# senyuanfan/inr-for-audio

Measured on AMD Instinct MI355X. Metric: coord-samples/sec trained, SIREN 5×1024 bf16 at 1/2/4/8 MI355X; recon SNR dB, higher is better.
Workload: dtype fp16

## Files before the change

include/siren_hip.h:

```cpp
#ifndef SIREN_HIP_H
#define SIREN_HIP_H

#include <stddef.h>
#include <stdint.h>

#ifdef __cplusplus
extern "C" {
#endif

#define SIREN_ABI_VERSION 12
#define SIREN_MAX_INNER 16
#define SIREN_MAX_HIDDEN 4096
#define SIREN_ROW_TILE 128
#define SIREN_TILEQ_INTS 768

enum siren_status {
  SIREN_OK = 0,
  SIREN_ERR_SHAPE = 1001,
  SIREN_ERR_NULL = 1002,
  SIREN_ERR_CONFIG = 1003
};

int siren_abi_version(void);
const char* siren_build_id(void);
int64_t siren_struct_size(int32_t which);
const char* siren_status_string(int status);

typedef struct siren_opt_state {
  double lr, best, step;
  int32_t num_bad, last_epoch;
  double min_lr, factor, threshold, eps_lr;
  int32_t patience, pad0;
  double beta1, beta2, eps;
} siren_opt_state;

typedef struct siren_guard {
  int32_t flag;
// ... 272 lines not shown
                          void* stream);
int siren_kan_regrid_refit(const double* gram, int32_t in, int32_t out, int32_t g_old, int32_t g_new,
                           const float* spline_w, const float* scaler, float* spline_w_new, int32_t* status,
                           void* stream);
int64_t siren_kan_grid_pass_rows(int32_t in);
int64_t siren_kan_grid_workspace_bytes(int64_t rows, int32_t in);
int siren_kan_grid_knots(const float* q, int32_t in, double margin, double grid_eps, float* grid_new, void* stream);
int siren_kan_grid_gram(const float* x, int64_t rows, int32_t in, const float* grid_old, const float* grid_new,
                        int32_t accumulate, double* gram, void* ws, void* stream);
int siren_kan_grid_refit(const double* gram, int32_t in, int32_t out, const float* spline_w, const float* scaler,
                         float* spline_w_new, int32_t* status, void* ws, void* stream);

enum siren_prof_kind {
  SIREN_PROF_FIRST_FWD = 0, SIREN_PROF_INNER_FWD = 1, SIREN_PROF_HEAD = 2, SIREN_PROF_BWD_DW = 3,
  SIREN_PROF_BWD_DX = 4, SIREN_PROF_BWD_DX0 = 5, SIREN_PROF_REDUCE = 6, SIREN_PROF_UPDATE = 7,
  SIREN_PROF_KAN_FWD = 8, SIREN_PROF_KAN_DW = 9, SIREN_PROF_KAN_DX = 10, SIREN_PROF_KAN_MISC = 11,
  SIREN_PROF_HEAD_FWD = 12,
  SIREN_PROF_LOSS = 13,
  SIREN_PROF_NKINDS = 14
};
enum siren_option {
  SIREN_OPT_NT_TILE = 0, SIREN_OPT_TN_TILE = 1, SIREN_OPT_NT_PIPE = 2, SIREN_OPT_TN_PIPE = 3,
  SIREN_OPT_NT_GRID = 4, SIREN_OPT_NT_DIAG = 6, SIREN_OPT_NT_QUEUE = 8, SIREN_OPT_HEAD_FUSE = 9,
  SIREN_OPT_HB_FAULT = 10, SIREN_OPT_KAN_GENERAL = 11
};
int siren_set_option(int32_t option, int32_t value);
int siren_profile_enable(int32_t max_records);
int siren_profile_reset(void);
int siren_profile_mask(uint32_t kinds);
int siren_profile_read(int32_t kind, double* total_ms, int64_t* count);

#ifdef __cplusplus
}
#endif
#endif
```

inr-for-audio_amd/_lib.py:

```python
from __future__ import annotations

import contextlib
import ctypes
import enum
import os

import torch

_HERE = os.path.dirname(os.path.abspath(__file__))
LIB_PATH = os.path.join(_HERE, "libsiren_hip.so")
ABI_VERSION = 12
MAX_INNER = 16
MAX_HIDDEN = 4096
ROW_TILE = 128
TILEQ_INTS = 768
ACT_SINE, ACT_SNAKE, ACT_TANH = 0, 1, 2
FP32_IDENTITY, FP32_SIN, FP32_TANH, FP32_SNAKE = 0, 1, 2, 3

_p = ctypes.c_void_p
_f32p = ctypes.POINTER(ctypes.c_float)
_i32 = ctypes.c_int32
_i64 = ctypes.c_int64


class SirenOptState(ctypes.Structure):
    _fields_ = [
        ("lr", ctypes.c_double), ("best", ctypes.c_double), ("step", ctypes.c_double),
        ("num_bad", _i32), ("last_epoch", _i32),
        ("min_lr", ctypes.c_double), ("factor", ctypes.c_double),
        ("threshold", ctypes.c_double), ("eps_lr", ctypes.c_double),
        ("patience", _i32), ("pad0", _i32),
        ("beta1", ctypes.c_double), ("beta2", ctypes.c_double), ("eps", ctypes.c_double),
    ]


class SirenGuard(ctypes.Structure):
    _fields_ = [("flag", _i32), ("headroom", _i32), ("clean", _i32), ("overflows", _i32),
                ("headroom0", _i32), ("stalls", _i32)]
# ... 255 lines not shown
    for k, st in enumerate(STRUCTS):
        if lib.siren_struct_size(k) != ctypes.sizeof(st):
            raise SirenError(f"{st.__name__}: ctypes size {ctypes.sizeof(st)} != C size {lib.siren_struct_size(k)}")
    return lib


def check(status: int, what: str = "siren") -> None:
    if status != 0:
        msg = load().siren_status_string(status)
        raise SirenError(f"{what} failed with status {status}: {msg.decode() if msg else '?'}")


class Opt(enum.IntEnum):
    NT_TILE = 0
    TN_TILE = 1
    NT_PIPE = 2
    TN_PIPE = 3
    NT_GRID = 4
    NT_DIAG = 6
    NT_QUEUE = 8
    HEAD_FUSE = 9
    HB_FAULT = 10
    KAN_GENERAL = 11


OPT_DEFAULTS = {Opt.NT_TILE: 0, Opt.TN_TILE: 0, Opt.NT_PIPE: -1, Opt.TN_PIPE: -1, Opt.NT_GRID: 0,
                Opt.NT_DIAG: 0, Opt.NT_QUEUE: 1, Opt.HEAD_FUSE: 1, Opt.HB_FAULT: 0, Opt.KAN_GENERAL: 0}


def _opt_shadow(lib) -> dict:
    return lib.__dict__.setdefault("_opt_shadow", dict(OPT_DEFAULTS))


def set_option(lib, opt, value: int) -> None:
    opt = Opt(opt)
    check(lib.siren_set_option(opt, value), f"siren_set_option({opt.name}, {value})")
    _opt_shadow(lib)[opt] = value


@contextlib.contextmanager
def options(lib, values: dict):
    shadow = _opt_shadow(lib)
    with contextlib.ExitStack() as undo:
        for opt, value in values.items():
            before = shadow[Opt(opt)]
            set_option(lib, opt, value)
            undo.callback(set_option, lib, opt, before)
        yield


# ... 11 lines not shown
```

inr-for-audio_amd/csrc/capi.hip:

```cpp
#include <string.h>
#include <vector>
#include "../../include/siren_hip.h"
#include "siren_kernels.h"

using namespace siren;

static_assert(sizeof(siren_opt_state) == sizeof(OptState), "opt state layout");
static_assert(sizeof(siren_guard) == sizeof(GuardState), "guard layout");
static_assert(SIREN_TILEQ_INTS == kTileqInts, "tile-queue set size");
static_assert(SIREN_MAX_INNER == siren::kMaxInner, "max hidden layers");
static_assert((int)SIREN_FP32_SNAKE == (int)siren::FP32_SNAKE && (int)SIREN_FP32_SIN == (int)siren::FP32_SIN &&
                  (int)SIREN_FP32_TANH == (int)siren::FP32_TANH, "fp32 act codes");

namespace {

inline hipStream_t S(void* s) { return (hipStream_t)s; }
inline const h16* B(const uint16_t* p) { return (const h16*)p; }
inline h16* B(uint16_t* p) { return (h16*)p; }

#define SIREN_TRY(expr)                        \
  do {                                         \
    const hipError_t _e = (expr);              \
    if (_e != hipSuccess) return (int)_e;      \
  } while (0)
// ... 39 lines not shown
bool hidden_ok(int h) {
  return (h >= 128 && h % 128 == 0 && h <= 1024 && 256 % (h / 4) == 0) || (h > 1024 && h % 1024 == 0 && h <= SIREN_MAX_HIDDEN);
}

bool rows_hidden_ok(int rows, int hidden, int row_mult = SIREN_ROW_TILE) {
  return hidden_ok(hidden) && rows > 0 && rows % row_mult == 0;
}

NtParams hidden_gemm(const h16* X, const h16* W, int rows, int hidden) {
  NtParams p = {};
  p.X = X;
  p.W = W;
  p.M = rows; p.N = hidden; p.K = hidden;
  p.tile = nt_choose_tile(rows, hidden);
  return p;
}

inline int bands(int rows) { return (rows + 255) / 256; }
inline int head_parts(int rows, int hidden) { return hidden / nt_choose_tile(rows, hidden); }
inline float loss_gfac(int loss_mode, double n_total) { return (float)((loss_mode == 1 ? 1.0 : 2.0) / n_total); }

template <class Grads, class Batch>
hipError_t zero_grads(const Grads* gr, const Batch* b, hipStream_t s) {
  if (!b->zero_grads || !gr->flat) return hipSuccess;
  return hipMemsetAsync(gr->flat, 0, gr->flat_len * sizeof(float), s);
}

int check_net(const siren_net* n) {
  if (!n) return SIREN_ERR_NULL;
  if (n->in_dim < 1 || n->in_dim > 2) return SIREN_ERR_CONFIG;
  if (!hidden_ok(n->hidden)) return SIREN_ERR_SHAPE;
  if (n->n_inner < 1 || n->n_inner > SIREN_MAX_INNER) return SIREN_ERR_CONFIG;
  if (!n->W0 || !n->b0 || !n->w_head || !n->b_head) return SIREN_ERR_NULL;
  for (int i = 0; i < n->n_inner; ++i) {
    if (!n->b[i] || !n->Wh[i] || !n->WTh[i]) return SIREN_ERR_NULL;
    if (n->act[i] < SIREN_ACT_SINE || n->act[i] > SIREN_ACT_TANH) return SIREN_ERR_CONFIG;
    if (n->act[i] == SIREN_ACT_SNAKE && !n->a[i]) return SIREN_ERR_NULL;
  }
  if (n->first_snake && !n->a0) return SIREN_ERR_NULL;
  if (!(n->head_omega >= 0.f)) return SIREN_ERR_CONFIG;
  if (n->rff_freq != 0) {
    if (n->rff_freq < 1 || n->rff_freq > kRffMaxFreq || n->in_dim != 1) return SIREN_ERR_CONFIG;
    if (!n->rff_B) return SIREN_ERR_NULL;
  }
  return SIREN_OK;
}

// ... 31 lines not shown
  }
  if (b->loss_mode < 0 || b->loss_mode > 2) return SIREN_ERR_CONFIG;
  if (sp && !(sp->alpha >= 0.0 && sp->alpha <= 1.0)) return SIREN_ERR_CONFIG;
  if (loss_step && spectral(b, sp)) {
    if (!sp || !sp->stft_ws || (sp->alpha != 0.0 && !sp->stft_basis)) return SIREN_ERR_NULL;
    if (b->n_total != (double)b->n_valid) return SIREN_ERR_CONFIG;
    if (b->n_valid < 1 || b->n_valid > kStftMaxN || (sp->alpha != 0.0 && spec_frames(kind, b->n_valid, 0) < 1))
      return SIREN_ERR_SHAPE;
  }
  return SIREN_OK;
}

inline hipError_t mark_ready(const siren_batch* b, int k, hipStream_t s) {
  return b->grad_ready[k] ? hipEventRecord((hipEvent_t)b->grad_ready[k], s) : hipSuccess;
}

inline void seg_add(ColSegs& sg, const float* src, float* out, int out_stride = 1) {
  if (sg.n < kMaxColSegs) {
    sg.src[sg.n] = src;
    sg.out[sg.n] = out;
    sg.out_stride[sg.n] = out_stride;
  }
  ++sg.n;
}

int hb_mode(int act) {
  return act == SIREN_ACT_SNAKE ? NT_FWD_HB_SNAKE : (act == SIREN_ACT_TANH ? NT_FWD_HB_TANH : NT_FWD_HB);
}
bool head_fused(const siren_net* n, const siren_batch* b, hipStream_t s) {
  const int act = n->act[n->n_inner - 1];
  if (!tuning().head_fuse || (act == SIREN_ACT_SNAKE && !b->head_scale_prev)) return false;
  if (!b->guard) return false;
  return gemm_nt_head_fusable(b->rows, n->hidden, s, hb_mode(act));
}

hipError_t run_forward(const siren_net* n, siren_batch* b, hipStream_t s, bool hb = false, float gfac = 0.f) {
  const int R = b->rows, H = n->hidden, L = n->n_inner;
  if (n->rff_freq > 0) {
    SIREN_PROF(SIREN_PROF_FIRST_FWD, s, rff_first_fwd(b->coords, n->rff_B, n->rff_freq, n->W0, n->b0, n->omega0, R, H,
                                                      B(b->Y[0]), B(b->C[0]), n->first_snake ? n->a0 : nullptr,
                                                      n->first_snake ? B(b->E[0]) : nullptr, B(b->enc), s));
  } else {
    SIREN_PROF(SIREN_PROF_FIRST_FWD, s, first_fwd(b->coords, n->in_dim, n->W0, n->b0, n->omega0, R, H, B(b->Y[0]),
                                                  B(b->C[0]), s, n->first_snake ? n->a0 : nullptr,
                                                  n->first_snake ? B(b->E[0]) : nullptr));
  }
  int run = 0;
  auto close_run = [&]() {
    if (run > 0) prof_end(s, run);
    run = 0;
  };
  for (int i = 0; i < L; ++i) {
    NtParams p = hidden_gemm(B(b->Y[i]), B(n->Wh[i]), R, H);
    p.omega = n->omega;
    p.bias = n->b[i];
    p.Y = B(b->Y[i + 1]);
    p.C = B(b->C[i + 1]);
    p.E = B(b->E[i + 1]);
    p.act_a = n->a[i];
    const bool head = (i == L - 1);
    p.head_w = n->w_head;
    p.head_part = b->head_part;
    p.tileq = b->tileq;
    if (head && hb) {
      p.target = b->target; p.b_head = n->b_head; p.out = b->out; p.g = b->g;
      p.sse_part = b->sse_part; p.gsum_part = b->gsum_part;
      p.n_valid = b->n_valid; p.loss_mode = b->loss_mode; p.gfac = gfac; p.head_omega = n->head_omega;
      p.gscale = b->gscale; p.dZ = B(b->dZ[0]); p.colsum_part = b->col_part;
      p.gmax_part = b->gmax_part;
      p.stall = b->guard ? &((GuardState*)b->guard)->stalls : nullptr;
      close_run();
      SIREN_PROF(SIREN_PROF_HEAD_FWD, s, gemm_nt(hb_mode(n->act[i]), true, p, s));
      continue;
    }
    if (run == 0) prof_begin(SIREN_PROF_INNER_FWD, s);
    const hipError_t e = gemm_nt(fwd_mode(n->act[i]), head, p, s);
    if (e != hipSuccess) {
      close_run();
      return e;
    }
    if (g_prof.open) ++run;
  }
  close_run();
  return hipSuccess;
}

}

extern "C" {

int siren_abi_version(void) { return SIREN_ABI_VERSION; }
// ... 73 lines not shown
static hipError_t rff_first_grads(bool fs, float omega0, int F, int R, int H, int prow, const h16* enc,
                                  const h16* dZ0, const float* gscale, const float* part, float* red_tmp,
                                  float* slab, float* gW0, float* gb0, float* ga0, hipStream_t s) {
  float* db = slab + rff_slab_floats(R, H, F) - H;
  ColSegs sg = {};
  if (fs) {
    seg_add(sg, part, gb0);
    seg_add(sg, part + H, ga0);
    SIREN_PROF(SIREN_PROF_REDUCE, s, col_reduce_multi(sg, 2 * (int64_t)H, prow, H, 1, red_tmp, s));
  } else {
    seg_add(sg, part, db);
    SIREN_PROF(SIREN_PROF_REDUCE, s, col_reduce_multi(sg, H, prow, H, 0, red_tmp, s));
  }
  SIREN_PROF(SIREN_PROF_BWD_DW, s, rff_dw0(enc, dZ0, F, R, H, fs ? 1.0f : omega0, gscale, slab, fs ? nullptr : db,
                                            gW0, gb0, s));
  return hipSuccess;
}

static int run_backward(const siren_net* net, const siren_grads* gr, siren_batch* b, hipStream_t s,
                        bool hb = false) {
  const int R = b->rows, H = net->hidden, L = net->n_inner, in = net->in_dim;
  const int ntile = nt_choose_tile(R, H), tntile = tn_choose_tile(R, H, H);
  const int prow = R / ntile;
  if (hb) {
    const bool snake_last = net->act[L - 1] == SIREN_ACT_SNAKE;
    ColSegs sg = {};
    seg_add(sg, b->col_part + H, gr->w_head);
    seg_add(sg, b->col_part, gr->b[L - 1]);
    if (snake_last) seg_add(sg, b->col_part + 2 * H, gr->a[L - 1]);
    SIREN_PROF(SIREN_PROF_REDUCE, s, col_reduce_multi(sg, (snake_last ? 3 : 2) * H, prow, H, 1, b->red_tmp, s));
  } else {
    const bool snake_last = net->act[L - 1] == SIREN_ACT_SNAKE;
    float* da_last = b->col_part + (int64_t)(R / 128) * H;
    SIREN_PROF(SIREN_PROF_HEAD, s, last_grad_scale(net, b, s));
    SIREN_PROF(SIREN_PROF_HEAD, s, head_bwd(B(b->C[L]), B(b->Y[L]), b->g, net->w_head, act_omega(net, L - 1),
                                            R, H, b->gscale, B(b->dZ[0]), b->col_part, b->col_part2,
                                            snake_last ? B(b->E[L]) : nullptr, snake_last ? da_last : nullptr, s));
    ColSegs sg = {};
    seg_add(sg, b->col_part2, gr->w_head);
    seg_add(sg, b->col_part, gr->b[L - 1]);
    if (snake_last) seg_add(sg, da_last, gr->a[L - 1]);
    SIREN_PROF(SIREN_PROF_REDUCE, s, col_reduce_multi(sg, H, R / 128, H, 1, b->red_tmp, s));
  }
  SIREN_TRY(mark_ready(b, L + 1, s));

  int cur = 0;
  for (int i = L - 1; i >= 0; --i) {
    TnParams tp = {};
    tp.Y = B(b->Y[i]);
    tp.dZ = B(b->dZ[cur]);
    tp.R = R; tp.Hin = H; tp.Hout = H;
    tp.splits = b->splits;
    tp.tile = tntile;
    tp.slab = b->slab;
    SIREN_PROF(SIREN_PROF_BWD_DW, s, gemm_tn_dw(tp, s));
    SIREN_PROF(SIREN_PROF_REDUCE, s, dw_reduce(b->slab, b->splits, H, H, tntile, gr->W[i], 1,
                                                       b->gscale, s));
    SIREN_TRY(mark_ready(b, i, s));

    NtParams p = hidden_gemm(B(b->dZ[cur]), B(net->WTh[i]), R, H);
    p.colsum_part = b->col_part;
    p.gscale = b->gscale;
    p.tileq = b->tileq;
    if (i > 0 || net->rff_freq > 0) {
      const bool snake = i > 0 ? net->act[i - 1] == SIREN_ACT_SNAKE : net->first_snake != 0;
      p.omega = i > 0 ? act_omega(net, i - 1) : 1.0f;
      p.Cprev = B(b->C[i]);
      p.Eprev = B(b->E[i]);
      p.dZ = B(b->dZ[cur ^ 1]);
      SIREN_PROF(i > 0 ? SIREN_PROF_BWD_DX : SIREN_PROF_BWD_DX0, s,
                 gemm_nt(snake ? NT_DX_SNAKE : NT_DX, false, p, s));
      if (i > 0) {
        const int64_t rs = (int64_t)(snake ? 2 : 1) * H;
        ColSegs sg = {};
        seg_add(sg, b->col_part, gr->b[i - 1]);
        if (snake) seg_add(sg, b->col_part + H, gr->a[i - 1]);
        SIREN_PROF(SIREN_PROF_REDUCE, s, col_reduce_multi(sg, rs, prow, H, 1, b->red_tmp, s));
        cur ^= 1;
      } else {
        SIREN_TRY(rff_first_grads(snake, net->omega0, net->rff_freq, R, H, prow, B(b->enc), B(b->dZ[cur ^ 1]),
                                  b->gscale, b->col_part, b->red_tmp, b->rff_slab, gr->W0, gr->b0, gr->a0, s));
        SIREN_TRY(mark_ready(b, L, s));
      }
    } else {
      const bool fs = net->first_snake != 0;
      p.omega = fs ? 1.0f : net->omega0;
      p.Cprev = B(b->C[0]);
      p.Eprev = B(b->E[0]);
      p.t = b->coords;
      p.in_dim = in;
      SIREN_PROF(SIREN_PROF_BWD_DX0, s, gemm_nt(fs ? NT_DX0_SNAKE : NT_DX0, false, p, s));
      const int64_t rs = (int64_t)(fs ? 2 + in : 1 + in) * H;
      ColSegs sg = {};
      if (fs) seg_add(sg, b->col_part + (int64_t)(1 + in) * H, gr->a0);
      seg_add(sg, b->col_part, gr->b0);
      for (int j = 0; j < in; ++j) seg_add(sg, b->col_part + (int64_t)(1 + j) * H, gr->W0 + j, in);
      SIREN_PROF(SIREN_PROF_REDUCE, s, col_reduce_multi(sg, rs, prow, H, 1, b->red_tmp, s));
      SIREN_TRY(mark_ready(b, L, s));
    }
  }
  return SIREN_OK;
}

static int backward_from_g(const siren_net* net, const siren_grads* gr, siren_batch* b, hipStream_t s) {
  const int R = b->rows;
  if (net->head_omega > 0.f)
    SIREN_TRY(head_sine_chain(b->head_part, head_parts(R, net->hidden), R, net->b_head, net->head_omega, b->g, s));
  SIREN_TRY(sum_to(b->g, R, gr->b_head, 1, s));
  SIREN_TRY(gmax_partials(b->g, R, b->gmax_part, s));
  return run_backward(net, gr, b, s);
}

static int run_spectral_step(const siren_net* net, const siren_grads* gr, siren_batch* b, const siren_spectral* sp,
                             SpecLoss kind, float gfac, hipStream_t s) {
  const int R = b->rows, n = b->n_valid;
  const bool stft = sp->alpha != 0.0, mr = kind == SPEC_MRSTFT;
  const SpecWs w = spec_ws_map(kind, sp->stft_ws, n, R);
  SIREN_TRY(run_forward(net, b, s));
  SIREN_PROF(SIREN_PROF_HEAD, s, head_loss(b->head_part, head_parts(R, net->hidden), R, net->b_head, b->target, n, gfac,
                                           b->out, b->g, b->sse_part, b->gsum_part, b->gmax_part, s, net->head_omega,
                                           b->loss_mode == 1 ? 1 : 0));
  if (b->loss_mode == 2) SIREN_PROF(SIREN_PROF_LOSS, s, snr_sums(b->out, b->target, n, w, s));
  if (stft) SIREN_PROF(SIREN_PROF_LOSS, s, spec_forward(b->out, n, sp->stft_basis, w, false, s));
// ... 662 lines not shown
constexpr bool kDiagBuild = false;
#endif

struct OptionRow {
  int id;
  int Tuning::*member;
  int def;
  bool (*accepts)(int);
  bool diag_only;
};
bool tile_ok(int v) { return v == 0 || v == 128 || v == 256; }
bool not_negative(int v) { return v >= 0; }
const OptionRow kOptions[] = {
    {SIREN_OPT_NT_TILE, &Tuning::nt_tile, 0, tile_ok, false},
    {SIREN_OPT_TN_TILE, &Tuning::tn_tile, 0, tile_ok, false},
    {SIREN_OPT_NT_PIPE, &Tuning::nt_pipe, -1, [](int v) { return v == -1 || v == 0 || v == 1 || (v >= 4 && v <= 7); }, false},
    {SIREN_OPT_TN_PIPE, &Tuning::tn_pipe, -1, [](int v) { return v >= -1 && v <= 4; }, false},
    {SIREN_OPT_NT_GRID, &Tuning::nt_grid, 0, not_negative, false},
    {SIREN_OPT_NT_DIAG, &Tuning::nt_diag, 0, [](int v) { return v >= 0 && !(v & ~(1 | 4 | 8 | 512 | 1024 | 2048)); }, true},
    {SIREN_OPT_NT_QUEUE, &Tuning::nt_queue, 1, [](int v) { return v >= 0 && v <= 2; }, false},
    {SIREN_OPT_HEAD_FUSE, &Tuning::head_fuse, 1, [](int v) { return v == 0 || v == 1; }, false},
    {SIREN_OPT_HB_FAULT, &Tuning::hb_fault, 0, not_negative, true},
    {SIREN_OPT_KAN_GENERAL, &Tuning::kan_general, 0, [](int v) { return v == 0 || v == 1; }, false},
};

Tuning default_tuning() {
  Tuning t{};
  for (const OptionRow& r : kOptions) t.*r.member = r.def;
  return t;
}

}

Tuning& siren::tuning() {
  static Tuning t = default_tuning();
  return t;
}

extern "C" {

int siren_set_option(int32_t option, int32_t value) {
  for (const OptionRow& r : kOptions) {
    if (r.id != option) continue;
    if (!r.accepts(value) || (r.diag_only && value && !kDiagBuild)) return SIREN_ERR_CONFIG;
    tuning().*r.member = value;
    return SIREN_OK;
// ... 342 lines not shown
```

inr-for-audio_amd/csrc/elementwise.hip:

```cpp
#include <math.h>
#include "siren_common.h"
#include "siren_kernels.h"

namespace siren {

static inline int grid_for(int64_t n, int per_block, int cap = 8192) {
  int64_t g = (n + per_block - 1) / per_block;
  if (g < 1) g = 1;
  if (g > cap) g = cap;
  return (int)g;
}

__global__ void coords_fill_kernel(float* t, int64_t rows, int64_t offset, int64_t n_total) {
  const float step = (n_total > 1) ? 2.0f / (float)(n_total - 1) : 0.f;
  const int64_t half = n_total / 2;
  for (int64_t r = (int64_t)blockIdx.x * blockDim.x + threadIdx.x; r < rows;
       r += (int64_t)gridDim.x * blockDim.x) {
    const int64_t i = offset + r;
    float v;
    if (i >= n_total) v = 0.f;
    else if (n_total == 1) v = -1.0f;
    else if (i < half) v = __builtin_fmaf(step, (float)i, -1.0f);
    else v = __builtin_fmaf(-step, (float)(n_total - 1 - i), 1.0f);
    t[r] = v;
// ... 378 lines not shown
    col_reduce_block(sg.src[z], row_stride, nrows, ncols, sg.out[z], 0, sg.out_stride[z], accumulate);
  else if (pass == 1)
    col_reduce_block(sg.src[z], row_stride, nrows, ncols, tz, ncols, 1, 0);
  else
    col_reduce_block(tz, ncols, 64, ncols, sg.out[z], 0, sg.out_stride[z], accumulate);
}

hipError_t col_reduce_multi(const ColSegs& sg, int64_t row_stride, int nrows, int ncols, int accumulate, float* tmp,
                            hipStream_t s) {
  if (sg.n < 1 || sg.n > kMaxColSegs) return hipErrorInvalidValue;
  const int cb = (ncols + 63) / 64;
  if (nrows <= 256) {
    hipLaunchKernelGGL(col_reduce_kernel, dim3(cb, 1, sg.n), dim3(256), 0, s, sg, row_stride, nrows, ncols, 0,
                       tmp, accumulate);
    return hipGetLastError();
  }
  hipLaunchKernelGGL(col_reduce_kernel, dim3(cb, 64, sg.n), dim3(256), 0, s, sg, row_stride, nrows, ncols, 1, tmp,
                     0);
  hipLaunchKernelGGL(col_reduce_kernel, dim3(cb, 1, sg.n), dim3(256), 0, s, sg, row_stride, nrows, ncols, 2, tmp,
                     accumulate);
  return hipGetLastError();
}

hipError_t col_reduce(const float* part, int64_t row_stride, int nrows, int ncols, float* out,
                      int out_stride, int accumulate, float* tmp, hipStream_t s) {
  ColSegs sg = {};
  sg.n = 1;
  sg.src[0] = part;
  sg.out[0] = out;
  sg.out_stride[0] = out_stride;
  return col_reduce_multi(sg, row_stride, nrows, ncols, accumulate, tmp, s);
}

__global__ void sum_to_kernel(const float* __restrict__ x, int n, float* out, int accumulate) {
  __shared__ float scratch[16];
  float s = 0.f;
  for (int i = threadIdx.x; i < n; i += blockDim.x) s += x[i];
  s = block_sum(s, scratch);
  if (threadIdx.x == 0) out[0] = accumulate ? out[0] + s : s;
}

hipError_t sum_to(const float* x, int n, float* out, int accumulate, hipStream_t s) {
  hipLaunchKernelGGL(sum_to_kernel, dim3(1), dim3(1024), 0, s, x, n, out, accumulate);
  return hipGetLastError();
}

// ... 153 lines not shown
```

inr-for-audio_amd/csrc/gemm_tn.hip:

```cpp
#include "gemm_pipeline.h"
#include "siren_common.h"
#include "siren_kernels.h"

namespace siren {

template <int BI_, int BJ_, int WM_, int WN_, int BK_ = 64, int S_ = 2, int PP_ = 0>
struct TnCfg {
  static constexpr int BI = BI_, BJ = BJ_, BK = BK_, S = S_;
  static constexpr int PP = PP_;
  static constexpr int WM = WM_, WN = WN_, NWAVES = WM_ * WN_, THREADS = 64 * NWAVES;
  static constexpr int TI = BI / WM, TJ = BJ / WN, SI = TI / 16, SJ = TJ / 16;
  static constexpr int YROW = BI * 2, ZROW = BJ * 2;
  static constexpr int YBYTES = BK * YROW, ZBYTES = BK * ZROW;
  static constexpr int STAGE = YBYTES + ZBYTES, LDS = S * STAGE;
  static constexpr int YINSTR = YBYTES / 1024 / NWAVES, ZINSTR = ZBYTES / 1024 / NWAVES;
  static constexpr int TILE_FLOATS = BI * BJ;
  static_assert(YBYTES % (1024 * NWAVES) == 0 && ZBYTES % (1024 * NWAVES) == 0, "staging split");
  static_assert(LDS <= 160 * 1024, "LDS");
};
using TnSmall = TnCfg<128, 128, 2, 2>;
using TnLarge = TnCfg<256, 256, 2, 4>;
using TnL0 = TnCfg<256, 256, 2, 4, 64, 2>;
using TnL1 = TnCfg<256, 256, 2, 4, 32, 4>;
using TnL2 = TnCfg<256, 256, 2, 4, 32, 5>;
// ... 205 lines not shown
  const int grid = (p.Hin / Cfg::BI) * (p.Hout / Cfg::BJ) * p.splits;
  hipLaunchKernelGGL(gemm_tn_kernel<Cfg>, dim3(grid), dim3(Cfg::THREADS), 0, s, p);
  return hipGetLastError();
}

hipError_t gemm_tn_dw(const TnParams& p, hipStream_t s) {
  if (p.Hin % 128 || p.Hout % 128 || p.R % 64 || p.R <= 0 || p.splits < 1) return hipErrorInvalidValue;
  if (p.tile == 256) {
    if (p.Hin % 256 || p.Hout % 256) return hipErrorInvalidValue;
    switch (tuning().tn_pipe >= 0 ? tuning().tn_pipe : 4) {
      case 0: return launch_tn<TnL0>(p, s);
      case 1: return (p.R % 32) ? hipErrorInvalidValue : launch_tn<TnL1>(p, s);
      case 2: return launch_tn<TnL2>(p, s);
      case 3: return launch_tn<TnLPP>(p, s);
      case 4: return launch_tn<TnLPP2>(p, s);
    }
    return hipErrorInvalidValue;
  }
  if (p.tile != 128) return hipErrorInvalidValue;
  return launch_tn<TnSmall>(p, s);
}

template <class Cfg>
__global__ void dw_reduce_kernel(const float4* __restrict__ slab, int splits, int Hin, int Hout,
                                 float* __restrict__ grad, int accumulate,
                                 const float* __restrict__ gscale) {
  constexpr int SUB = Cfg::SI * Cfg::SJ;
  const float inv = gscale ? gscale[1] : 1.0f;
  const int tiles_j = Hout / Cfg::BJ;
  const int ntile = (Hin / Cfg::BI) * tiles_j;
  constexpr int TQ = Cfg::TILE_FLOATS / 4;
  const int64_t total = (int64_t)ntile * TQ;
  for (int64_t q = (int64_t)blockIdx.x * blockDim.x + threadIdx.x; q < total;
       q += (int64_t)gridDim.x * blockDim.x) {
    constexpr int U = 16;
    float4 w[U];
    const int n1 = splits < U ? splits : U;
#pragma unroll
    for (int u = 0; u < U; ++u)
      if (u < n1) w[u] = slab[q + (int64_t)u * total];
    float4 v = w[0];
#pragma unroll
    for (int u = 1; u < U; ++u)
      if (u < n1) { v.x += w[u].x; v.y += w[u].y; v.z += w[u].z; v.w += w[u].w; }
    for (int s = n1; s < splits; s += U) {
      const int n = splits - s < U ? splits - s : U;
#pragma unroll
      for (int u = 0; u < U; ++u)
        if (u < n) w[u] = slab[q + (int64_t)(s + u) * total];
// ... 2 lines not shown
        if (u < n) { v.x += w[u].x; v.y += w[u].y; v.z += w[u].z; v.w += w[u].w; }
    }
    v.x *= inv; v.y *= inv; v.z *= inv; v.w *= inv;
    const int tile = (int)(q / TQ);
    const int within = (int)(q - (int64_t)tile * TQ);
    const int lane = within & 63, blk = within >> 6;
    const int ij = blk % SUB, wave = blk / SUB;
    const int i = ij / Cfg::SJ, j = ij % Cfg::SJ;
    const int wm = wave / Cfg::WN, wn = wave % Cfg::WN;
    const int ti = tile / tiles_j, tj = tile - ti * tiles_j;
    const int k = ti * Cfg::BI + wm * Cfg::TI + i * 16 + 4 * (lane >> 4);
    const int o = tj * Cfg::BJ + wn * Cfg::TJ + j * 16 + (lane & 15);
    float4* out = (float4*)(grad + (size_t)o * Hin + k);
    if (accumulate) {
      float4 a = *out;
      a.x += v.x; a.y += v.y; a.z += v.z; a.w += v.w;
      *out = a;
    } else {
      *out = v;
    }
  }
}

hipError_t dw_reduce(const float* slab, int splits, int Hin, int Hout, int tile, float* grad,
                     int accumulate, const float* gscale, hipStream_t s) {
  const int64_t total = (int64_t)Hin * Hout / 4;
  int grid = (int)((total + 63) / 64);
  if (grid > 8192) grid = 8192;
  if (tile == 256) {
    hipLaunchKernelGGL(dw_reduce_kernel<TnLarge>, dim3(grid), dim3(64), 0, s, (const float4*)slab, splits,
                       Hin, Hout, grad, accumulate, gscale);
  } else if (tile == 128) {
    hipLaunchKernelGGL(dw_reduce_kernel<TnSmall>, dim3(grid), dim3(64), 0, s, (const float4*)slab, splits,
                       Hin, Hout, grad, accumulate, gscale);
  } else {
    return hipErrorInvalidValue;
  }
  return hipGetLastError();
}

}
```

inr-for-audio_amd/csrc/siren_kernels.h:

```cpp
#pragma once
#include <hip/hip_runtime.h>
#include <stdint.h>

namespace siren {

typedef _Float16 h16;

enum NtMode { NT_FWD = 0, NT_DX = 1, NT_DX0 = 2, NT_FWD_SNAKE = 3, NT_FWD_TANH = 4, NT_DX_SNAKE = 5,
              NT_DX0_SNAKE = 6, NT_FWD_HB = 7, NT_FWD_HB_SNAKE = 8, NT_FWD_HB_TANH = 9 };
constexpr bool nt_is_hb(int m) { return m == NT_FWD_HB || m == NT_FWD_HB_SNAKE || m == NT_FWD_HB_TANH; }
constexpr bool nt_is_fwd(int m) { return m == NT_FWD || m == NT_FWD_SNAKE || m == NT_FWD_TANH || nt_is_hb(m); }
constexpr bool nt_is_snake_fwd(int m) { return m == NT_FWD_SNAKE || m == NT_FWD_HB_SNAKE; }

struct Tuning {
  int nt_tile, tn_tile;
  int nt_pipe, tn_pipe;
  int nt_grid;
  int nt_diag;
  int nt_queue;
  int head_fuse;
  int hb_fault;
  int kan_general;
};
Tuning& tuning();

struct NtParams {
  const h16* X;
  const h16* W;
  int M, N, K;
  int ld;
  int tile;
  float omega;
  const float* bias;
  h16* Y;
  h16* C;
  h16* E;
  const float* act_a;
  const float* head_w;
  float* head_part;
  const h16* Cprev;
  const h16* Eprev;
  h16* dZ;
  float* colsum_part;
  const float* t;
  int in_dim;
  const float* gscale;
  int diag;
  int* tileq;
  const float* target;
  const float* b_head;
  float* out;
  float* g;
  float* sse_part;
  float* gsum_part;
  int n_valid, loss_mode;
  float gfac, head_omega;
  float* gmax_part;
  int* stall;
  int spin_limit, hb_fault;
};
constexpr int kTileqInts = 768;

int nt_choose_tile(int M, int N);
hipError_t gemm_nt(int mode, bool head, const NtParams& p, hipStream_t s);
bool gemm_nt_one_ok(const NtParams& p);
hipError_t gemm_nt_one(const NtParams& p, int grid, int diag, bool overlap, hipStream_t s);
bool gemm_nt_big_ok(const NtParams& p);
hipError_t gemm_nt_big(const NtParams& p, int grid, int diag, hipStream_t s);
bool gemm_nt_head_fusable(int M, int N, hipStream_t s, int mode = NT_FWD_HB);
struct TnParams {
  const h16* Y;
  const h16* dZ;
  int R, Hin, Hout;
  int splits;
  int tile;
  float* slab;
};

int tn_choose_tile(int R, int Hin, int Hout);
hipError_t gemm_tn_dw(const TnParams& p, hipStream_t s);
hipError_t dw_reduce(const float* slab, int splits, int Hin, int Hout, int tile, float* grad,
                     int accumulate, const float* gscale, hipStream_t s);

hipError_t coords_fill(float* t, int64_t rows, int64_t offset, int64_t n_total, hipStream_t s);
hipError_t coords_fill_grid(float* xy, int64_t rows, int64_t offset, int64_t height, int width, hipStream_t s);

struct GuardState {
  int32_t flag, headroom, clean, overflows, headroom0;
  int32_t stalls;
};
constexpr int kHeadroomDefault = 6;
constexpr int kHeadroomDrop = 4;
constexpr int kHeadroomMin = -14;
constexpr int kHeadroomGrowAfter = 1000;
__device__ __forceinline__ bool guard_overflow(const GuardState* g, const float* sse) {
  return g && g->flag && __builtin_isfinite(sse[0]) && g->headroom > kHeadroomMin;
}
__device__ __forceinline__ bool guard_stalled(const GuardState* g) { return g && g->stalls != 0; }
__device__ __forceinline__ bool guard_skip(const GuardState* g, const float* sse) {
  return guard_stalled(g) || guard_overflow(g, sse);
}
hipError_t guard_check(const float* g, int64_t n, GuardState* guard, hipStream_t s, const float* sse = nullptr);
hipError_t first_fwd(const float* t, int in_dim, const float* W0, const float* b0, float omega0,
                     int R, int H, h16* Y0, h16* C0, hipStream_t s, const float* a0 = nullptr,
                     h16* E0 = nullptr);
// ... 3 lines not shown
                     int loss_mode = 0);
hipError_t gmax_partials(const float* g, int R, float* gmax_part, hipStream_t s);
hipError_t head_sine_chain(const float* head_part, int nparts, int R, const float* b_head, float omega, float* g,
                           hipStream_t s);
hipError_t grad_scale_bound(const float* ymax_part, int nparts, const float* w_head, const float* b_head, int H,
                            float gfac, float head_omega, int loss_mode, float act_bound, float* gscale,
                            hipStream_t s, const GuardState* guard = nullptr);
hipError_t grad_scale(const float* gmax_part, int nparts, const float* w_head, int H, float omega,
                      float* gscale, hipStream_t s, const GuardState* guard = nullptr);
hipError_t head_bwd(const h16* C, const h16* Y, const float* g, const float* w_head, float omega,
                    int R, int H, const float* gscale, h16* dZ, float* db_part, float* dwh_part,
                    const h16* E, float* da_part, hipStream_t s);
hipError_t col_reduce(const float* part, int64_t row_stride, int nrows, int ncols, float* out,
                      int out_stride, int accumulate, float* tmp, hipStream_t s);
constexpr int kMaxColSegs = 4;
struct ColSegs {
  const float* src[kMaxColSegs];
  float* out[kMaxColSegs];
  int out_stride[kMaxColSegs];
  int n;
};
hipError_t col_reduce_multi(const ColSegs& sg, int64_t row_stride, int nrows, int ncols, int accumulate, float* tmp,
                            hipStream_t s);

enum Fp32Act { FP32_IDENTITY = 0, FP32_SIN = 1, FP32_TANH = 2, FP32_SNAKE = 3 };
hipError_t fp32_linear(const float* x, int64_t rows, int in, int out, const float* W, const float* b, float omega,
                       float* pre, hipStream_t s);
hipError_t fp32_act(int act, const float* x, int64_t rows, int cols, const float* a, float* y, hipStream_t s);
hipError_t fp32_act_bwd(int act, const float* x, int64_t rows, int cols, const float* a, const float* gy,
                        float* gpre, float* da_prod, hipStream_t s);
hipError_t fp32_linear_bwd(const float* x, int64_t rows, int in, int out, const float* W, float omega, float* gpre,
                           float* gx, float* gW, float* gb, float* slab, int splits, float* tmp, hipStream_t s);

constexpr int kRffMaxFreq = 256;
int rff_kpad(int F);
int rff_splits(int R, int H, int F);
int64_t rff_slab_floats(int R, int H, int F);
hipError_t rff_encode(const float* x, const float* Bf, int F, int64_t rows, float* out, hipStream_t s);
hipError_t rff_encode16(const float* x, const float* Bf, int F, int R, h16* enc, hipStream_t s);
hipError_t rff_first_fwd(const float* x, const float* Bf, int F, const float* W0, const float* b0, float omega0, int R,
                         int H, h16* Y0, h16* C0, const float* a0, h16* E0, h16* enc, hipStream_t s);
hipError_t rff_dw0(const h16* enc, const h16* dZ0, int F, int R, int H, float scale, const float* gscale,
                   float* slab, const float* db, float* gW0, float* gb0, hipStream_t s);

enum SpecLoss { SPEC_STFT = 0, SPEC_MRSTFT = 1 };
constexpr int kStftMinN = 512, kMrRes = 3, kMrMinN = 1024, kMrScalFloats = 32;
// ... 82 lines not shown
int64_t kan_regrid_pass_rows(int in, int Go, int Gn);
int64_t kan_regrid_part_doubles(int64_t N, int in, int Go, int Gn);
hipError_t kan_regrid_gram(const float* X, const float* grid_old, const float* grid_new, int64_t N, int in, int Go,
                           int Gn, int accumulate, double* part, double* gram, hipStream_t s);
hipError_t kan_regrid_refit(const double* gram, int in, int out, int Go, int Gn, const float* spline_w,
                            const float* scaler, float* spline_w_new, int* status, hipStream_t s);

struct OptState {
  double lr;
  double best;
  double step;
  int32_t num_bad;
  int32_t last_epoch;
  double min_lr, factor, threshold, eps_lr;
  int32_t patience, pad0;
  double beta1, beta2, eps;
};

hipError_t adam_flat(float* p, const float* g, float* m, float* v, int64_t n, const OptState* st,
                     hipStream_t s, const GuardState* guard = nullptr, const float* sse = nullptr);
hipError_t plateau_step(OptState* st, const float* sse, double n_total, float* loss_hist,
                        double* lr_hist, int64_t hist_cap, hipStream_t s, GuardState* guard = nullptr);
hipError_t cast_weight(const float* W, int H_out, int H_in, h16* Wb, h16* WTb, hipStream_t s);
constexpr int kMaxInner = 16;
struct CastSet {
  const float* W[kMaxInner];
  h16* Wb[kMaxInner];
  h16* WTb[kMaxInner];
  int n;
};
hipError_t cast_weights(const CastSet& cs, int H, hipStream_t s);

struct PlaneSet {
  int64_t w_off[kMaxInner];
  h16* Wb[kMaxInner];
  h16* WTb[kMaxInner];
  int64_t lo[kMaxInner + 1], hi[kMaxInner + 1];
  int n, nrest;
};
hipError_t plane_point(const float* theta, const float* d1, const float* d2, float a, float b, float* out,
                       const PlaneSet& ps, int H, hipStream_t s);
hipError_t plane_loss(const float* sse_part, int nparts, double* slot, hipStream_t s);
hipError_t sum_to(const float* x, int n, float* out, int accumulate, hipStream_t s);
hipError_t sum_to2(const float* x0, float* out0, const float* x1, float* out1, int n, int accumulate, hipStream_t s,
                   const int* flag_src = nullptr, float* flag_dst = nullptr);

}
// ... 1 lines not shown
```

inr-for-audio_amd/engine.py:

```python
from __future__ import annotations

import ctypes
import math
from dataclasses import dataclass

import torch

from . import _lib
from ._lib import (MAX_INNER, ROW_TILE, SirenBatch, SirenGrads, SirenKanBatch, SirenNet, SirenOptState, check,
                   ptr)

SEG_ALIGN = 64
STORE16 = torch.float16


def round_up(x: int, m: int) -> int:
    return (x + m - 1) // m * m


@dataclass
class NetSpec:
    in_dim: int
    hidden: int
    n_inner: int
# ... 69 lines not shown
                [e(R, H, dtype=h) if spec.act(i) == _lib.ACT_SNAKE else None for i in range(L)]
        else:
            ping = [e(R, H, dtype=h), e(R, H, dtype=h)]
            scratch = e(R, H, dtype=h)
            self.Y = [ping[i % 2] for i in range(L + 1)]
            self.C = [scratch] * (L + 1)
            snake = spec.first_snake or any(spec.act(i) == _lib.ACT_SNAKE for i in range(L))
            escr = e(R, H, dtype=h) if snake else None
            self.E = [escr if spec.first_snake else None] + \
                [escr if spec.act(i) == _lib.ACT_SNAKE else None for i in range(L)]
        self.out = e(R)
        self.g = torch.zeros(R, dtype=f32, device=device)
        self.head_part = e(H // 128, R)
        nsum = (R + 255) // 256
        self.sse_part = e(nsum)
        self.gsum_part = e(nsum)
        self.gmax_part = e(nsum)
        self.gscale = torch.ones(2, dtype=f32, device=device)
        self.tileq = _lib.new_tileq(device)
        self.train = train
        if train:
            self.splits = int(splits or lib.siren_default_splits(R, H))
            self.dZ = [e(R, H, dtype=h) for _ in range(2)]
            self.col_part = e(R // 128, max(2 + spec.in_dim, 2), H)
            self.col_part2 = e(R // 128, H)
            self.red_tmp = e(4, 64, H)
            self.slab = e(int(lib.siren_slab_floats(H, self.splits)))
        else:
            self.splits = 1
            self.dZ = [None, None]
            self.col_part = self.col_part2 = self.red_tmp = self.slab = None
        self.enc = self.rff_slab = None
        if train and spec.rff_freq:
            self.enc = torch.zeros(R, int(lib.siren_rff_kpad(spec.rff_freq)), dtype=h, device=device)
            self.rff_slab = e(int(lib.siren_rff_slab_floats(R, H, spec.rff_freq)))

    def batch(self, coords: torch.Tensor, target, n_valid: int, n_total: float,
              zero_grads: bool = False, guard: torch.Tensor | None = None, loss_mode: int = 0) -> SirenBatch:
        b = SirenBatch()
        b.rows, b.n_valid, b.n_total = self.rows, int(n_valid), float(n_total)
        b.splits, b.zero_grads = self.splits, int(zero_grads)
        b.guard, b.loss_mode = ptr(guard), int(loss_mode)
        b.coords, b.target = ptr(coords), ptr(target)
        for i, y in enumerate(self.Y):
            b.Y[i] = ptr(y)
        for i, c in enumerate(self.C):
            b.C[i] = ptr(c)
        for i, x in enumerate(self.E):
            b.E[i] = ptr(x)
        b.dZ[0], b.dZ[1] = ptr(self.dZ[0]), ptr(self.dZ[1])
        b.out, b.g, b.head_part = ptr(self.out), ptr(self.g), ptr(self.head_part)
        b.sse_part, b.gsum_part = ptr(self.sse_part), ptr(self.gsum_part)
        b.gmax_part, b.gscale = ptr(self.gmax_part), ptr(self.gscale)
        b.col_part, b.col_part2 = ptr(self.col_part), ptr(self.col_part2)
        b.red_tmp, b.slab = ptr(self.red_tmp), ptr(self.slab)
        b.tileq = ptr(self.tileq)
        b.enc, b.rff_slab = ptr(self.enc), ptr(self.rff_slab)
        return b


def make_net(spec: NetSpec, W0, b0, bs, Whs, WThs, w_head, b_head, snake_a=None, a0=None, rff_B=None) -> SirenNet:
    n = SirenNet()
    n.in_dim, n.hidden, n.n_inner = spec.in_dim, spec.hidden, spec.n_inner
    n.omega0, n.omega = spec.omega0, spec.omega
# ... 717 lines not shown
```

Before: 42.32 million.

## Defer and batch backward column and dW reductions into single multi-segment launches

Backward no longer launches a column-reduction and a dW-reduction kernel per layer. Each layer's partial sums go to its own region of enlarged col_part and slab buffers, and after the backward loop one batched col_reduce kernel and one dw_reduce_multi kernel (grid over layers) finish them all. This cuts kernel-launch and serialization overhead and gives the reduction kernels more parallel work. In exchange it uses more scratch memory, and gradients are finalized later, so it is turned off when per-layer grad_ready signalling (multi-device overlap) is in use. The feature is enabled by a flag packed into zero_grads.

```diff
diff --git a/include/siren_hip.h b/include/siren_hip.h
--- a/include/siren_hip.h
+++ b/include/siren_hip.h
@@ -13,6 +13,7 @@
 #define SIREN_MAX_HIDDEN 4096
 #define SIREN_ROW_TILE 128
 #define SIREN_TILEQ_INTS 768
+#define SIREN_BATCH_REDUCE_WS 2
 
 enum siren_status {
   SIREN_OK = 0,
@@ -331,7 +332,7 @@
 enum siren_option {
   SIREN_OPT_NT_TILE = 0, SIREN_OPT_TN_TILE = 1, SIREN_OPT_NT_PIPE = 2, SIREN_OPT_TN_PIPE = 3,
   SIREN_OPT_NT_GRID = 4, SIREN_OPT_NT_DIAG = 6, SIREN_OPT_NT_QUEUE = 8, SIREN_OPT_HEAD_FUSE = 9,
-  SIREN_OPT_HB_FAULT = 10, SIREN_OPT_KAN_GENERAL = 11
+  SIREN_OPT_HB_FAULT = 10, SIREN_OPT_KAN_GENERAL = 11, SIREN_OPT_BATCH_REDUCE = 12
 };
 int siren_set_option(int32_t option, int32_t value);
 int siren_profile_enable(int32_t max_records);
diff --git a/inr-for-audio_amd/_lib.py b/inr-for-audio_amd/_lib.py
--- a/inr-for-audio_amd/_lib.py
+++ b/inr-for-audio_amd/_lib.py
@@ -14,6 +14,7 @@
 MAX_HIDDEN = 4096
 ROW_TILE = 128
 TILEQ_INTS = 768
+BATCH_REDUCE_WS = 2
 ACT_SINE, ACT_SNAKE, ACT_TANH = 0, 1, 2
 FP32_IDENTITY, FP32_SIN, FP32_TANH, FP32_SNAKE = 0, 1, 2, 3
 
@@ -315,10 +316,12 @@
     HEAD_FUSE = 9
     HB_FAULT = 10
     KAN_GENERAL = 11
+    BATCH_REDUCE = 12
 
 
 OPT_DEFAULTS = {Opt.NT_TILE: 0, Opt.TN_TILE: 0, Opt.NT_PIPE: -1, Opt.TN_PIPE: -1, Opt.NT_GRID: 0,
-                Opt.NT_DIAG: 0, Opt.NT_QUEUE: 1, Opt.HEAD_FUSE: 1, Opt.HB_FAULT: 0, Opt.KAN_GENERAL: 0}
+                Opt.NT_DIAG: 0, Opt.NT_QUEUE: 1, Opt.HEAD_FUSE: 1, Opt.HB_FAULT: 0, Opt.KAN_GENERAL: 0,
+                Opt.BATCH_REDUCE: 3}
 
 
 def _opt_shadow(lib) -> dict:
diff --git a/inr-for-audio_amd/csrc/capi.hip b/inr-for-audio_amd/csrc/capi.hip
--- a/inr-for-audio_amd/csrc/capi.hip
+++ b/inr-for-audio_amd/csrc/capi.hip
@@ -85,7 +85,7 @@
 
 template <class Grads, class Batch>
 hipError_t zero_grads(const Grads* gr, const Batch* b, hipStream_t s) {
-  if (!b->zero_grads || !gr->flat) return hipSuccess;
+  if (!(b->zero_grads & 1) || !gr->flat) return hipSuccess;
   return hipMemsetAsync(gr->flat, 0, gr->flat_len * sizeof(float), s);
 }
 
@@ -163,6 +163,36 @@
     sg.out_stride[sg.n] = out_stride;
   }
   ++sg.n;
+}
+
+inline int64_t part_rows(int R, int H) { return (int64_t)(R / 128) * H; }
+int batch_bits(const siren_net* n, const siren_batch* b) {
+  if (!(b->zero_grads & SIREN_BATCH_REDUCE_WS)) return 0;
+  for (int k = 0; k < n->n_inner + 2; ++k)
+    if (b->grad_ready[k]) return 0;
+  return tuning().batch_reduce;
+}
+float* head_parts_at(const siren_net* n, const siren_batch* b) {
+  const int first = n->in_dim + 2 > 2 ? n->in_dim + 2 : 2;
+  return b->col_part + ((batch_bits(n, b) & 1) ? first * part_rows(b->rows, n->hidden) : 0);
+}
+float* stage_parts_at(const siren_net* n, const siren_batch* b, int i) {
+  if (!(batch_bits(n, b) & 1)) return b->col_part;
+  return head_parts_at(n, b) + (3 + 2 * (int64_t)(i - 1)) * part_rows(b->rows, n->hidden);
+}
+float* slab_at(const siren_net* n, const siren_batch* b, int i) {
+  if (!(batch_bits(n, b) & 2)) return b->slab;
+  return b->slab + (int64_t)i * siren_slab_floats(n->hidden, b->splits);
+}
+void batch_add(ColBatch& cb, const ColSegs& sg, int64_t row_stride, int nrows) {
+  for (int z = 0; z < sg.n; ++z, ++cb.n) {
+    if (cb.n >= kMaxBatchSegs) continue;
+    cb.src[cb.n] = sg.src[z];
+    cb.out[cb.n] = sg.out[z];
+    cb.out_stride[cb.n] = sg.out_stride[z];
+    cb.row_stride[cb.n] = row_stride;
+    cb.nrows[cb.n] = nrows;
+  }
 }
 
 int hb_mode(int act) {
@@ -207,7 +237,7 @@
       p.target = b->target; p.b_head = n->b_head; p.out = b->out; p.g = b->g;
       p.sse_part = b->sse_part; p.gsum_part = b->gsum_part;
       p.n_valid = b->n_valid; p.loss_mode = b->loss_mode; p.gfac = gfac; p.head_omega = n->head_omega;
-      p.gscale = b->gscale; p.dZ = B(b->dZ[0]); p.colsum_part = b->col_part;
+      p.gscale = b->gscale; p.dZ = B(b->dZ[0]); p.colsum_part = head_parts_at(n, b);
       p.gmax_part = b->gmax_part;
       p.stall = b->guard ? &((GuardState*)b->guard)->stalls : nullptr;
       close_run();
@@ -327,25 +357,36 @@
   const int R = b->rows, H = net->hidden, L = net->n_inner, in = net->in_dim;
   const int ntile = nt_choose_tile(R, H), tntile = tn_choose_tile(R, H, H);
   const int prow = R / ntile;
+  const int bits = batch_bits(net, b);
+  ColBatch cbat = {};
+  DwSet dws = {};
+  auto reduce_cols = [&](const ColSegs& sg, int64_t rs, int nrows) -> hipError_t {
+    if (bits & 1) {
+      batch_add(cbat, sg, rs, nrows);
+      return hipSuccess;
+    }
+    SIREN_PROF(SIREN_PROF_REDUCE, s, col_reduce_multi(sg, rs, nrows, H, 1, b->red_tmp, s));
+    return hipSuccess;
+  };
+  const bool snake_last = net->act[L - 1] == SIREN_ACT_SNAKE;
+  float* hp = head_parts_at(net, b);
   if (hb) {
-    const bool snake_last = net->act[L - 1] == SIREN_ACT_SNAKE;
     ColSegs sg = {};
-    seg_add(sg, b->col_part + H, gr->w_head);
-    seg_add(sg, b->col_part, gr->b[L - 1]);
-    if (snake_last) seg_add(sg, b->col_part + 2 * H, gr->a[L - 1]);
-    SIREN_PROF(SIREN_PROF_REDUCE, s, col_reduce_multi(sg, (snake_last ? 3 : 2) * H, prow, H, 1, b->red_tmp, s));
+    seg_add(sg, hp + H, gr->w_head);
+    seg_add(sg, hp, gr->b[L - 1]);
+    if (snake_last) seg_add(sg, hp + 2 * H, gr->a[L - 1]);
+    SIREN_TRY(reduce_cols(sg, (snake_last ? 3 : 2) * H, prow));
   } else {
-    const bool snake_last = net->act[L - 1] == SIREN_ACT_SNAKE;
-    float* da_last = b->col_part + (int64_t)(R / 128) * H;
+    float* da_last = hp + (int64_t)(R / 128) * H;
     SIREN_PROF(SIREN_PROF_HEAD, s, last_grad_scale(net, b, s));
     SIREN_PROF(SIREN_PROF_HEAD, s, head_bwd(B(b->C[L]), B(b->Y[L]), b->g, net->w_head, act_omega(net, L - 1),
-                                            R, H, b->gscale, B(b->dZ[0]), b->col_part, b->col_part2,
+                                            R, H, b->gscale, B(b->dZ[0]), hp, b->col_part2,
                                             snake_last ? B(b->E[L]) : nullptr, snake_last ? da_last : nullptr, s));
     ColSegs sg = {};
     seg_add(sg, b->col_part2, gr->w_head);
-    seg_add(sg, b->col_part, gr->b[L - 1]);
+    seg_add(sg, hp, gr->b[L - 1]);
     if (snake_last) seg_add(sg, da_last, gr->a[L - 1]);
-    SIREN_PROF(SIREN_PROF_REDUCE, s, col_reduce_multi(sg, H, R / 128, H, 1, b->red_tmp, s));
+    SIREN_TRY(reduce_cols(sg, H, R / 128));
   }
   SIREN_TRY(mark_ready(b, L + 1, s));
 
@@ -357,14 +398,18 @@
     tp.R = R; tp.Hin = H; tp.Hout = H;
     tp.splits = b->splits;
     tp.tile = tntile;
-    tp.slab = b->slab;
+    tp.slab = slab_at(net, b, i);
     SIREN_PROF(SIREN_PROF_BWD_DW, s, gemm_tn_dw(tp, s));
-    SIREN_PROF(SIREN_PROF_REDUCE, s, dw_reduce(b->slab, b->splits, H, H, tntile, gr->W[i], 1,
-                                                       b->gscale, s));
+    if (bits & 2) {
+      dws.slab[dws.n] = tp.slab;
+      dws.grad[dws.n++] = gr->W[i];
+    } else {
+      SIREN_PROF(SIREN_PROF_REDUCE, s, dw_reduce(tp.slab, b->splits, H, H, tntile, gr->W[i], 1, b->gscale, s));
+    }
     SIREN_TRY(mark_ready(b, i, s));
 
     NtParams p = hidden_gemm(B(b->dZ[cur]), B(net->WTh[i]), R, H);
-    p.colsum_part = b->col_part;
+    p.colsum_part = i > 0 ? stage_parts_at(net, b, i) : b->col_part;
     p.gscale = b->gscale;
     p.tileq = b->tileq;
     if (i > 0 || net->rff_freq > 0) {
@@ -378,9 +423,9 @@
       if (i > 0) {
         const int64_t rs = (int64_t)(snake ? 2 : 1) * H;
         ColSegs sg = {};
-        seg_add(sg, b->col_part, gr->b[i - 1]);
-        if (snake) seg_add(sg, b->col_part + H, gr->a[i - 1]);
-        SIREN_PROF(SIREN_PROF_REDUCE, s, col_reduce_multi(sg, rs, prow, H, 1, b->red_tmp, s));
+        seg_add(sg, p.colsum_part, gr->b[i - 1]);
+        if (snake) seg_add(sg, p.colsum_part + H, gr->a[i - 1]);
+        SIREN_TRY(reduce_cols(sg, rs, prow));
         cur ^= 1;
       } else {
         SIREN_TRY(rff_first_grads(snake, net->omega0, net->rff_freq, R, H, prow, B(b->enc), B(b->dZ[cur ^ 1]),
@@ -400,10 +445,13 @@
       if (fs) seg_add(sg, b->col_part + (int64_t)(1 + in) * H, gr->a0);
       seg_add(sg, b->col_part, gr->b0);
       for (int j = 0; j < in; ++j) seg_add(sg, b->col_part + (int64_t)(1 + j) * H, gr->W0 + j, in);
-      SIREN_PROF(SIREN_PROF_REDUCE, s, col_reduce_multi(sg, rs, prow, H, 1, b->red_tmp, s));
+      SIREN_TRY(reduce_cols(sg, rs, prow));
       SIREN_TRY(mark_ready(b, L, s));
     }
   }
+  if (cbat.n > 0) SIREN_PROF(SIREN_PROF_REDUCE, s, col_reduce_batch(cbat, H, 1, b->red_tmp, s));
+  if (dws.n > 0)
+    SIREN_PROF(SIREN_PROF_REDUCE, s, dw_reduce_multi(dws, b->splits, H, H, tntile, 1, b->gscale, s));
   return SIREN_OK;
 }
 
@@ -1112,6 +1160,7 @@
     {SIREN_OPT_HEAD_FUSE, &Tuning::head_fuse, 1, [](int v) { return v == 0 || v == 1; }, false},
     {SIREN_OPT_HB_FAULT, &Tuning::hb_fault, 0, not_negative, true},
     {SIREN_OPT_KAN_GENERAL, &Tuning::kan_general, 0, [](int v) { return v == 0 || v == 1; }, false},
+    {SIREN_OPT_BATCH_REDUCE, &Tuning::batch_reduce, 3, [](int v) { return v >= 0 && v <= 3; }, false},
 };
 
 Tuning default_tuning() {
diff --git a/inr-for-audio_amd/csrc/elementwise.hip b/inr-for-audio_amd/csrc/elementwise.hip
--- a/inr-for-audio_amd/csrc/elementwise.hip
+++ b/inr-for-audio_amd/csrc/elementwise.hip
@@ -424,6 +424,30 @@
   return hipGetLastError();
 }
 
+__global__ void col_reduce_batch_kernel(ColBatch cb, int ncols, int pass, float* tmp, int accumulate) {
+  const int z = blockIdx.z;
+  const bool two = cb.nrows[z] > 256;
+  float* tz = tmp + (int64_t)z * 64 * ncols;
+  if (pass == 1) {
+    if (two) col_reduce_block(cb.src[z], cb.row_stride[z], cb.nrows[z], ncols, tz, ncols, 1, 0);
+  } else if (two) {
+    col_reduce_block(tz, ncols, 64, ncols, cb.out[z], 0, cb.out_stride[z], accumulate);
+  } else {
+    col_reduce_block(cb.src[z], cb.row_stride[z], cb.nrows[z], ncols, cb.out[z], 0, cb.out_stride[z], accumulate);
+  }
+}
+
+hipError_t col_reduce_batch(const ColBatch& cb, int ncols, int accumulate, float* tmp, hipStream_t s) {
+  if (cb.n < 1 || cb.n > kMaxBatchSegs) return hipErrorInvalidValue;
+  const int nb = (ncols + 63) / 64;
+  bool two = false;
+  for (int z = 0; z < cb.n; ++z) two = two || cb.nrows[z] > 256;
+  if (two)
+    hipLaunchKernelGGL(col_reduce_batch_kernel, dim3(nb, 64, cb.n), dim3(256), 0, s, cb, ncols, 1, tmp, 0);
+  hipLaunchKernelGGL(col_reduce_batch_kernel, dim3(nb, 1, cb.n), dim3(256), 0, s, cb, ncols, 2, tmp, accumulate);
+  return hipGetLastError();
+}
+
 hipError_t col_reduce(const float* part, int64_t row_stride, int nrows, int ncols, float* out,
                       int out_stride, int accumulate, float* tmp, hipStream_t s) {
   ColSegs sg = {};
diff --git a/inr-for-audio_amd/csrc/gemm_tn.hip b/inr-for-audio_amd/csrc/gemm_tn.hip
--- a/inr-for-audio_amd/csrc/gemm_tn.hip
+++ b/inr-for-audio_amd/csrc/gemm_tn.hip
@@ -251,9 +251,9 @@
 }
 
 template <class Cfg>
-__global__ void dw_reduce_kernel(const float4* __restrict__ slab, int splits, int Hin, int Hout,
-                                 float* __restrict__ grad, int accumulate,
-                                 const float* __restrict__ gscale) {
+__device__ __forceinline__ void dw_reduce_body(const float4* __restrict__ slab, int splits, int Hin, int Hout,
+                                               float* __restrict__ grad, int accumulate,
+                                               const float* __restrict__ gscale) {
   constexpr int SUB = Cfg::SI * Cfg::SJ;
   const float inv = gscale ? gscale[1] : 1.0f;
   const int tiles_j = Hout / Cfg::BJ;
@@ -302,6 +302,20 @@
   }
 }
 
+template <class Cfg>
+__global__ void dw_reduce_kernel(const float4* __restrict__ slab, int splits, int Hin, int Hout,
+                                 float* __restrict__ grad, int accumulate,
+                                 const float* __restrict__ gscale) {
+  dw_reduce_body<Cfg>(slab, splits, Hin, Hout, grad, accumulate, gscale);
+}
+
+template <class Cfg>
+__global__ void dw_reduce_multi_kernel(DwSet set, int splits, int Hin, int Hout, int accumulate,
+                                       const float* __restrict__ gscale) {
+  dw_reduce_body<Cfg>((const float4*)set.slab[blockIdx.y], splits, Hin, Hout, set.grad[blockIdx.y], accumulate,
+                      gscale);
+}
+
 hipError_t dw_reduce(const float* slab, int splits, int Hin, int Hout, int tile, float* grad,
                      int accumulate, const float* gscale, hipStream_t s) {
   const int64_t total = (int64_t)Hin * Hout / 4;
@@ -319,4 +333,22 @@
   return hipGetLastError();
 }
 
-}
+hipError_t dw_reduce_multi(const DwSet& set, int splits, int Hin, int Hout, int tile, int accumulate,
+                           const float* gscale, hipStream_t s) {
+  if (set.n < 1 || set.n > kMaxInner) return hipErrorInvalidValue;
+  const int64_t total = (int64_t)Hin * Hout / 4;
+  int grid = (int)((total + 63) / 64);
+  if (grid > 8192) grid = 8192;
+  if (tile == 256) {
+    hipLaunchKernelGGL(dw_reduce_multi_kernel<TnLarge>, dim3(grid, set.n), dim3(64), 0, s, set, splits, Hin, Hout,
+                       accumulate, gscale);
+  } else if (tile == 128) {
+    hipLaunchKernelGGL(dw_reduce_multi_kernel<TnSmall>, dim3(grid, set.n), dim3(64), 0, s, set, splits, Hin, Hout,
+                       accumulate, gscale);
+  } else {
+    return hipErrorInvalidValue;
+  }
+  return hipGetLastError();
+}
+
+}
diff --git a/inr-for-audio_amd/csrc/siren_kernels.h b/inr-for-audio_amd/csrc/siren_kernels.h
--- a/inr-for-audio_amd/csrc/siren_kernels.h
+++ b/inr-for-audio_amd/csrc/siren_kernels.h
@@ -21,6 +21,7 @@
   int head_fuse;
   int hb_fault;
   int kan_general;
+  int batch_reduce;
 };
 Tuning& tuning();
 
@@ -60,6 +61,7 @@
   int spin_limit, hb_fault;
 };
 constexpr int kTileqInts = 768;
+constexpr int kMaxInner = 16;
 
 int nt_choose_tile(int M, int N);
 hipError_t gemm_nt(int mode, bool head, const NtParams& p, hipStream_t s);
@@ -81,6 +83,13 @@
 hipError_t gemm_tn_dw(const TnParams& p, hipStream_t s);
 hipError_t dw_reduce(const float* slab, int splits, int Hin, int Hout, int tile, float* grad,
                      int accumulate, const float* gscale, hipStream_t s);
+struct DwSet {
+  const float* slab[kMaxInner];
+  float* grad[kMaxInner];
+  int n;
+};
+hipError_t dw_reduce_multi(const DwSet& set, int splits, int Hin, int Hout, int tile, int accumulate,
+                           const float* gscale, hipStream_t s);
 
 hipError_t coords_fill(float* t, int64_t rows, int64_t offset, int64_t n_total, hipStream_t s);
 hipError_t coords_fill_grid(float* xy, int64_t rows, int64_t offset, int64_t height, int width, hipStream_t s);
@@ -130,6 +139,16 @@
 };
 hipError_t col_reduce_multi(const ColSegs& sg, int64_t row_stride, int nrows, int ncols, int accumulate, float* tmp,
                             hipStream_t s);
+constexpr int kMaxBatchSegs = 3 + 2 * (kMaxInner - 1) + 4;
+struct ColBatch {
+  const float* src[kMaxBatchSegs];
+  float* out[kMaxBatchSegs];
+  int64_t row_stride[kMaxBatchSegs];
+  int nrows[kMaxBatchSegs];
+  int out_stride[kMaxBatchSegs];
+  int n;
+};
+hipError_t col_reduce_batch(const ColBatch& cb, int ncols, int accumulate, float* tmp, hipStream_t s);
 
 enum Fp32Act { FP32_IDENTITY = 0, FP32_SIN = 1, FP32_TANH = 2, FP32_SNAKE = 3 };
 hipError_t fp32_linear(const float* x, int64_t rows, int in, int out, const float* W, const float* b, float omega,
@@ -258,7 +277,6 @@
 hipError_t plateau_step(OptState* st, const float* sse, double n_total, float* loss_hist,
                         double* lr_hist, int64_t hist_cap, hipStream_t s, GuardState* guard = nullptr);
 hipError_t cast_weight(const float* W, int H_out, int H_in, h16* Wb, h16* WTb, hipStream_t s);
-constexpr int kMaxInner = 16;
 struct CastSet {
   const float* W[kMaxInner];
   h16* Wb[kMaxInner];
diff --git a/inr-for-audio_amd/engine.py b/inr-for-audio_amd/engine.py
--- a/inr-for-audio_amd/engine.py
+++ b/inr-for-audio_amd/engine.py
@@ -115,10 +115,10 @@
         if train:
             self.splits = int(splits or lib.siren_default_splits(R, H))
             self.dZ = [e(R, H, dtype=h) for _ in range(2)]
-            self.col_part = e(R // 128, max(2 + spec.in_dim, 2), H)
+            self.col_part = e(R // 128, max(2 + spec.in_dim, 2) + 3 + 2 * (L - 1), H)
             self.col_part2 = e(R // 128, H)
-            self.red_tmp = e(4, 64, H)
-            self.slab = e(int(lib.siren_slab_floats(H, self.splits)))
+            self.red_tmp = e(7 + 2 * (L - 1), 64, H)
+            self.slab = e(L * int(lib.siren_slab_floats(H, self.splits)))
         else:
             self.splits = 1
             self.dZ = [None, None]
@@ -132,7 +132,7 @@
               zero_grads: bool = False, guard: torch.Tensor | None = None, loss_mode: int = 0) -> SirenBatch:
         b = SirenBatch()
         b.rows, b.n_valid, b.n_total = self.rows, int(n_valid), float(n_total)
-        b.splits, b.zero_grads = self.splits, int(zero_grads)
+        b.splits, b.zero_grads = self.splits, int(zero_grads) | (_lib.BATCH_REDUCE_WS if self.train else 0)
         b.guard, b.loss_mode = ptr(guard), int(loss_mode)
         b.coords, b.target = ptr(coords), ptr(target)
         for i, y in enumerate(self.Y):
```

After: 42.34 million, median of 4. No clear change (+0.0%).
